# rockstaedt/DecentralOPF.jl

Measured on AMD Instinct MI355X. Metric: agent_subproblem_updates_per_sec, higher is better.
Workload: dtype f64

## Files before the change

decentralopf.jl_amd/csrc/dopf_api.hip:

```cpp
#include <algorithm>
#include <cmath>
#include <cstdarg>
#include <cstdio>
#include <cstdlib>
#include <cstring>
#include <numeric>
#include <string>
#include <vector>

#include "dopf_ctx.h"

using namespace dopf;

namespace {

#ifndef DOPF_UNROLL
#define DOPF_UNROLL 16
#endif
constexpr int kUnroll = DOPF_UNROLL, kMid = 4;
constexpr int kGraphIters[3] = {kUnroll, kMid, 1};
constexpr int kCheckEvery = 512;
thread_local char g_create_err[512];

}
// ... 318 lines not shown
};

Step make_step(const dopf_ctx *c, bool quiet, bool outside = false)
{
    const Plan &p = c->plan;
    const bool single = c->comm == nullptr && !outside;
    const XchgView *x = outside ? nullptr : comm_xchg(c);
    Step st{};
    st.xd = x && ((c->v.L == 0 && p.sliceDual) || c->tail_xchg) ? x : nullptr;
    st.like_single = single || st.xd != nullptr;
    st.comm_quiet = quiet && !st.like_single && x != nullptr && p.commQuiet;
    st.v = c->v;
    DevView &v = st.v;
    v.sliceDual = st.like_single && p.sliceDual;
    v.tail = st.like_single && c->v.tailDev && (c->comm == nullptr || c->tail_xchg) ? c->v.tailDev : nullptr;
    v.slackInDual = (st.like_single || st.comm_quiet) && p.slackDual;
    v.slackGlobal = st.comm_quiet ? 1 : 0;
    v.quiet = single && v.slackInDual && quiet;
    return st;
}

bool quiet_allowed(const dopf_ctx *c)
{
    return c->comm ? c->plan.commQuiet && comm_xchg(c) != nullptr && !c->tail_xchg : c->plan.quiet;
}

int settle_quiet(dopf_ctx *c, bool *parked)
{
    *parked = c->host_st.halt == 2;
    if (*parked) {
        HIPCHK(c, hipMemsetAsync(&c->v.st->halt, 0, sizeof(int), c->main));
        c->host_st.halt = 0;
        c->quiet = false;
        ++c->quiet_parked;
    } else if (!c->host_st.halt) {
        c->quiet = (c->comm ? c->plan.commQuiet : c->plan.quiet) && c->host_st.walk_last == 0;
    }
    return DOPF_OK;
}

enum { E_T0, E_T1, E_G0, E_G1, E_S0, E_S1, E_K0, E_K1, E_R1, E_D1, E_X0, E_X1, E_N };

void enqueue_local(dopf_ctx *c, const Step &st, const hipEvent_t *ev = nullptr)
{
    const DevView &v = st.v;
    const Plan &p = c->plan;
    auto mark = [&](int k, hipStream_t s) { if (ev) hipEventRecord(ev[k], s); };
    mark(E_T0, c->main);
    launch_tables(v, p, c->main);
    mark(E_T1, c->main);
    const bool fork = v.nGenItems > 0 && v.nStoItems > 0 && (c->q.flags & DOPF_F_OVERLAP_AGENTS);
    if (fork) {
        hipEventRecord(c->evFork, c->main);
        hipStreamWaitEvent(c->side, c->evFork, 0);
        mark(E_S0, c->side);
        launch_sto_update(v, p, c->side);
        mark(E_S1, c->side);
        hipEventRecord(c->evJoin, c->side);
    }
    mark(E_G0, c->main);
    if (p.fuseAgents) launch_agents_fused(v, p, c->main);
    else if (p.fuseNet) launch_net_agents(v, p, c->main);
    else launch_gen_update(v, p, c->main);
    mark(E_G1, c->main);
    if (fork) {
        hipStreamWaitEvent(c->main, c->evJoin, 0);
    } else {
        mark(E_S0, c->main);
        if (!p.fuseAgents && !p.fuseNet) launch_sto_update(v, p, c->main);
        mark(E_S1, c->main);
    }
    mark(E_K0, c->main);
    if (!v.tail && !v.quiet) launch_slack(v, c->main);
    mark(E_K1, c->main);
    if (!v.tail && !v.slackInDual) launch_reduce(v, p, c->main);
    mark(E_R1, c->main);
}

void enqueue_apply(dopf_ctx *c, const Step &st, const hipEvent_t *ev = nullptr)
{
    if (!st.v.tail) launch_dual(st.v, c->plan, c->main, st.xd);
    if (ev) for (int k : {E_D1, E_X0, E_X1}) hipEventRecord(ev[k], c->main);
}

int enqueue_iteration(dopf_ctx *c, bool quiet = false, const hipEvent_t *ev = nullptr)
{
    const Step st = make_step(c, quiet);
    enqueue_local(c, st, ev);
    if (st.comm_quiet) launch_xchg(c->v, *comm_xchg(c), c->main, true);
    else if (!st.like_single) { const int rc = comm_enqueue_allreduce(c); if (rc) return rc; }
    enqueue_apply(c, st, ev);
    return DOPF_OK;
}

int build_graph(dopf_ctx *c, int iters, hipGraphExec_t *out, bool quiet = false)
{
    hipGraph_t g = nullptr;
    HIPCHK(c, hipStreamBeginCapture(c->main, c->comm ? hipStreamCaptureModeThreadLocal : hipStreamCaptureModeRelaxed));
    int rc = DOPF_OK;
    for (int i = 0; i < iters && rc == DOPF_OK; ++i) rc = enqueue_iteration(c, quiet);
    const hipError_t ec = hipStreamEndCapture(c->main, &g);
    if (rc) { if (g) hipGraphDestroy(g); return rc; }
    if (ec != hipSuccess) return fail(c, DOPF_E_DEVICE, "hipStreamEndCapture: %s", hipGetErrorString(ec));
    hipError_t e = hipGraphInstantiate(out, g, nullptr, nullptr, 0);
    hipGraphDestroy(g);
    if (e != hipSuccess) return fail(c, DOPF_E_DEVICE, "hipGraphInstantiate: %s", hipGetErrorString(e));
    return DOPF_OK;
}

int build_graphs(dopf_ctx *c, bool quiet)
{
    dopf_ctx::Graphs &gs = c->graphs[quiet];
    for (int k = 0; k < 3; ++k)
        if (const int rc = build_graph(c, kGraphIters[k], &gs.g[k], quiet)) return rc;
    gs.valid = true;
// ... 292 lines not shown
        d.zeros(&v.part_U, NT * L); d.zeros(&v.part_K, NT * L); d.zeros(&v.node_dsum, NT);
        d.zeros(&v.walk_flag, LT); d.zeros(&v.walk_any, T); d.zeros(&v.tab_skip, T);
    }
    d.zeros(&v.part_ginj, (size_t)v.nGenItems * T); d.zeros(&v.part_gcost, v.nGenItems);
    d.zeros(&v.part_sinj, (size_t)v.nStoItems * T); d.zeros(&v.part_scost, v.nStoItems);
    d.zeros(&v.part_sinj_w, (size_t)v.nStoItems * T); d.zeros(&v.part_scost_w, v.nStoItems);
    if (L > 0) { d.upload(&v.row_of_pos, lo.row_of_pos); d.upload(&v.pos_of_row, lo.pos_of_row); }
    if (L > 0) d.zeros(&v.part_T, (size_t)v.rowsT * T);
    if (L > 0) d.zeros(&v.prev_node, NT);
    d.zeros(&v.nu_prev, (size_t)S * T); d.zeros(&v.nu_valid, S); d.zeros(&v.sto_fail, S);
    d.zeros(&v.item_fail, v.nStoItems);
    d.zeros(&v.part2, (size_t)N * v.reduceRB * T); d.zeros(&v.part2_cost, v.reduceRB);
    d.zeros(&v.reduce_ticket, (size_t)N * ((T + 31) / 32));
    d.zeros(&v.dual_ticket, 1);
    if (pl.tail) {
        d.zeros(&tvh.acc, (size_t)2 * kAccRep * tvh.accStride);
        tvh.expect = agent_blocks(v);
        TailView *tvd = nullptr;
        d.raw(&tvd, 1);
        if (d.rc) return d.rc;
        HIPCHK(c, hipMemcpy(tvd, &tvh, sizeof tvh, hipMemcpyHostToDevice));
        v.tailDev = tvd;
    }
    if (pl.wideNet) {
        std::vector<double> na(N);
        for (int n = 0; n < N; ++n)
            na[n] = (double)((lo.node_gen_beg[n + 1] - lo.node_gen_beg[n]) + (lo.node_sto_beg[n + 1] - lo.node_sto_beg[n]));
        d.upload(&v.node_na, na);
    }
    double *cons = nullptr;
    d.zeros(&cons, NT + 2 * LT + 1);
// ... 887 lines not shown
```

decentralopf.jl_amd/csrc/dopf_internal.h:

```cpp
#pragma once

#include <hip/hip_runtime.h>
#include <stddef.h>
#include <stdint.h>
#include <stdlib.h>

#include <type_traits>

#include "../../include/dopf.h"
#include "dopf_plan.h"
#include "ramp_dp.h"
#include "budget_root.h"
#include "central_rows.h"

namespace dopf {

struct Status {
    int iteration;
    int converged;
    int halt;
    int iters_total;
    unsigned long long solver_fail;
    unsigned long long dbg_scans, dbg_wave_loops, dbg_events;
    unsigned long long dbg_cyc[6];
    unsigned long long dbg_reason[4];
    unsigned long long resbits[3];
    unsigned long long resbits2[2][3];
    int walk_last;
    int res_set;
    double res[3];
    double total_cost;
    int xchg_timeout;
    int tail_timeout;
    int tail_par;
};

struct XchgView;
struct TailView {
    long long *acc;
    int accStride;
    int expect;
    double scaleInj, invInj, scaleCost, invCost;
    const XchgView *xchg;
};

struct DevView {
    const DevView *self;
    int N, L, T, G, S, M2;
    int maxNodeAgents;
    int nGenItems, nStoItems;
    int genTT, genR;
    int genRows;
// ... 197 lines not shown
void central_launch_iteration(const CentralView &c, const Plan &p, const DevView &vreduce, hipStream_t s);
void central_launch_metrics(const CentralView &c, const Plan &p, const DevView &vreduce, const double *XP, const double *XD, const double *XC,
                            const double *XE, const double *yb, const double *yf, const double *XR, const double *XQ, double scale, hipStream_t s);
void central_launch_scale_copy(double *dst, const double *src, double scale, size_t n, hipStream_t s);
constexpr int kCentralDiffBlocks = 256;
int central_diff_blocks(size_t n);
void central_launch_diff_sq(const double *a, const double *b, size_t n, double *part, hipStream_t s);
void central_launch_scale_copy_primal(const CentralView &c, const Plan &p, double scale, hipStream_t s);

inline int agent_blocks(const DevView &v) { return v.nStoItems + (v.genBlocks > 0 && !v.genSkip ? v.genBlocks : v.nGenItems); }

void launch_gen_update(const DevView &v, const Plan &p, hipStream_t s);
void launch_gen_ramp(const DevView &v, const Plan &p, hipStream_t s);
void launch_gen_ramp_net(const DevView &v, const Plan &p, hipStream_t s);
void launch_gen_budget(const DevView &v, const Plan &p, hipStream_t s);
void launch_sto_update(const DevView &v, const Plan &p, hipStream_t s);
void launch_net_agents(const DevView &v, const Plan &p, hipStream_t s);
void launch_agents_fused(const DevView &v, const Plan &p, hipStream_t s);
int debug_timeline(unsigned long long *out, int n);
hipError_t raise_lds_limits(const DevView &v, const Plan &p);
void launch_tables(const DevView &v, const Plan &p, hipStream_t s);
void launch_slack(const DevView &v, hipStream_t s);
void launch_reduce(const DevView &v, const Plan &p, hipStream_t s);
constexpr int kXchgMaxWorld = 16;
constexpr int kXchgChunk = 2048;
struct XchgView {
    int world, me, nchunks;
    int rs;
    unsigned long long n;
    unsigned long long timeout_ticks;
    double *data[kXchgMaxWorld];
    unsigned long long *flags[kXchgMaxWorld];
    double *sum[kXchgMaxWorld];
// ... 18 lines not shown
```

decentralopf.jl_amd/csrc/kernels_agents.hip:

```cpp
#include "dopf_internal.h"

namespace dopf {

#if defined(DOPF_STATS) || defined(DOPF_BLOCK_STAMPS)
__device__ unsigned long long g_timeline[8192 * 8 + 8192 * 8];
#endif
#if defined(DOPF_STATS) || defined(DOPF_BLOCK_STAMPS)
#define DOPF_BLOCK_ENTER() { if (threadIdx.x == 0 && blockIdx.x < 8192 * 4) g_timeline[32768 + 2 * blockIdx.x] = wall_clock64(); }
#define DOPF_BLOCK_EXIT() { __syncthreads(); if (threadIdx.x == 0 && blockIdx.x < 8192 * 4) g_timeline[32768 + 2 * blockIdx.x + 1] = wall_clock64(); }
#else
#define DOPF_BLOCK_ENTER()
#define DOPF_BLOCK_EXIT()
#endif
#ifdef DOPF_BLOCK_STAMPS
#define DOPF_TAIL_STAMP(i) { if (threadIdx.x == 0) g_timeline[(i)] = wall_clock64(); }
#else
#define DOPF_TAIL_STAMP(i)
#endif
#ifdef DOPF_STATS
#define DOPF_STAMP(i) { if (lane == 0 && rep == 0 && round == 0) { const int w_ = blk * 4 + (tid >> 6); if (w_ < 8192) g_timeline[w_ * 8 + (i)] = wall_clock64(); } }
#else
#define DOPF_STAMP(i)
#endif

// ... 141 lines not shown
            v.st->total_cost = ctot;
        }
    }
    for (int d = 32; d > 0; d >>= 1) rl = fmax(rl, __shfl_xor(rl, d));
    if ((tid & 63) == 0) wmaxT[tid >> 6] = rl;
    asm volatile("s_waitcnt lgkmcnt(0)\n\ts_barrier" ::: "memory");
    DOPF_TAIL_STAMP(3)
    if (tid == 0) {
        if (badT & 2) { v.st->xchg_timeout = 1; v.st->halt = 1; return; }
        if (badT) { v.st->tail_timeout = 1; v.st->halt = 1; return; }
        double r0 = 0.0;
        for (int q = 0; q < nth / 64; ++q) r0 = fmax(r0, wmaxT[q]);
        v.st->tail_par = par ^ 1;
        status_update(v, spre, r0, 0.0, 0.0);
    }
}

__device__ __forceinline__ void lin_coef(double w, double iw, double kap, double &ia, double &idet, double &s2)
{
    const double r2 = rcp64(w + 2.0 * kap);
    ia = rcp64(w + kap);
    idet = iw * r2;
    s2 = 2.0 * r2;
}

template <int BS, int FL = 4, bool AV = false, bool QC = false>
__device__ __forceinline__ void gen_lines_body(const DevView &v, const int item, const int TT, const int R)
{
    __shared__ double red[BS];
    const Item it = v.gen_items[item];
// ... 262 lines not shown
}

template <bool LINES, bool AV = false, bool QC = false>
__global__ __launch_bounds__(512) void k_gen_update(DevView v)
{
    gen_update_body<LINES, AV, QC>(v);
}

template <int BS, bool TAIL, bool LDS_ONLY = false>
__device__ __forceinline__ void gen_pair_sums(const DevView &v, const int blk, const int tid, const int r, const int tt,
                                              double acc0, double acc1, double cost, double (*red)[BS], double *wc)
{
    const int T = v.T, TT = v.genTT2, R = v.genR2;
    TailView tv{};
    int par = 0;
    if (TAIL) { tv = *v.tail; par = v.st->tail_par; }
    for (int d = 32; d > 0; d >>= 1) cost += __shfl_xor(cost, d);
    red[0][tid] = acc0; red[1][tid] = acc1;
    if ((tid & 63) == 0) wc[tid >> 6] = cost;
    if (LDS_ONLY) asm volatile("s_waitcnt lgkmcnt(0)\n\ts_barrier" ::: "memory");
    else __syncthreads();
    if (r == 0 && tt < TT) {
        double s0 = 0.0, s1 = 0.0;
        for (int q = 0; q < R; ++q) { s0 += red[0][q * TT + tt]; s1 += red[1][q * TT + tt]; }
        if (TAIL) {
            acc_add(tv, par, 2 * tt, s0, tv.scaleInj);
            acc_add(tv, par, 2 * tt + 1, s1, tv.scaleInj);
        } else {
            v.part_ginj[(size_t)blk * T + 2 * tt] = s0;
            v.part_ginj[(size_t)blk * T + 2 * tt + 1] = s1;
        }
// ... 14 lines not shown
    __shared__ double wc[BS / 64];
    Item it;
    if (v.genChunk > 0) { it.a0 = blk * v.genChunk; it.a1 = min(v.G, it.a0 + v.genChunk); it.node = 0; }
    else it = v.gen_items[blk];
    const int T = v.T, N = v.N, TT = v.genTT2, R = v.genR2;
    const int tid = threadIdx.x;
    const int r = tid / TT, tt = tid - r * TT;
    const double w = v.w_prox, gam = v.gamma;
    const double inv = 1.0 / (w + gam);
    double cost = 0.0, acc0 = 0.0, acc1 = 0.0;
    const double *ftab = nullptr;
    const int *prof = nullptr;
    if constexpr (AV) { ftab = *gen_avail_slot(v); prof = gen_prof(v); }
    if (r < R) {
        const int t = 2 * tt;
        const double sh0 = fma(gam, v.s[t], v.price[it.node + N * t]) * inv;
        const double sh1 = fma(gam, v.s[t + 1], v.price[it.node + N * (t + 1)]) * inv;
        double2 *P2 = reinterpret_cast<double2 *>(v.P);
        const size_t half = (size_t)(T >> 1);
        constexpr int GU = BS == 256 ? 6 : 4;
        for (int g0 = it.a0 + r; g0 < it.a1; g0 += GU * R) {
            double2 p0[GU], cp[GU];
            double mc[GU], pm[GU];
            int pr[GU];
#pragma unroll
            for (int u = 0; u < GU; ++u) {
                const int g = g0 + u * R < it.a1 ? g0 + u * R : g0;
                mc[u] = v.gen_mc[g]; pm[u] = v.gen_pmax[g];
                p0[u] = P2[(size_t)g * half + tt];
                if constexpr (AV) pr[u] = prof[g];
            }
            if constexpr (AV) {
// ... 19 lines not shown
}

template <int BS, bool TAIL, bool AV = false>
__device__ __forceinline__ bool gen_pair_stream(const DevView &v, const int first, const int stride)
{
    constexpr int GU = kGenStreamRows;
    __shared__ double red[2][BS];
    __shared__ double wc[BS / 64];
    const int halt = v.st->halt;
    const int T = v.T, N = v.N, TT = v.genTT2, R = v.genR2, nI = v.nGenItems, chunk = v.genChunk, G = v.G;
    const int tid = threadIdx.x;
    const int r = tid / TT, tt = tid - r * TT;
    const bool rowlane = r < R;
    const double gam = v.gamma, inv = 1.0 / (v.w_prox + gam);
    const int t2c = 2 * tt;
    const double sh0 = fma(gam, v.s[t2c], v.price[(size_t)N * t2c]) * inv;
    const double sh1 = fma(gam, v.s[t2c + 1], v.price[(size_t)N * (t2c + 1)]) * inv;
    if (first >= nI) return halt == 0;
    double2 *P2 = reinterpret_cast<double2 *>(v.P);
    const size_t half = (size_t)(T >> 1);
    double2 pa[GU], pb[GU];
    double mca[GU], pma[GU], mcb[GU], pmb[GU];
    int pra[GU], prb[GU];
    const double *ftab = nullptr;
    const int *prof = nullptr;
    if constexpr (AV) { ftab = *gen_avail_slot(v); prof = gen_prof(v); }
#define DOPF_GEN_LOAD(item, p, mc, pm, pr)                                                  \
    {                                                                                       \
        const int a0_ = (item) * chunk, a1_ = min(G, a0_ + chunk);                          \
        _Pragma("unroll") for (int u = 0; u < GU; ++u) {                                    \
            const int g_ = (rowlane && a0_ + r + u * R < a1_) ? a0_ + r + u * R : a0_;      \
            const double2 mp_ = v.gen_mp[g_];                                               \
// ... 56 lines not shown
__device__ __forceinline__ void gen_pair_skip_body(const DevView &v, const int blk)
{
    __shared__ double red[2][BS];
    __shared__ double wc[BS / 64], wlo[BS / 64], whi[BS / 64];
    __shared__ int flg[2][BS];
    const Item it = v.gen_items[blk];
    const int T = v.T, N = v.N, TT = v.genTT2, R = v.genR2;
    const int tid = threadIdx.x;
    const int r = tid / TT, tt = tid - r * TT;
    const double w = v.w_prox, gam = v.gamma;
    const double inv = 1.0 / (w + gam);
    double cost = 0.0, acc0 = 0.0, acc1 = 0.0;
    double sh0 = 0.0, sh1 = 0.0;
    if (r < R) {
        const int t = 2 * tt;
        sh0 = fma(gam, v.s[t], v.price[it.node + N * t]) * inv;
        sh1 = fma(gam, v.s[t + 1], v.price[it.node + N * (t + 1)]) * inv;
    }
    double lo = (r == 0 && tt < TT) ? fmin(sh0, sh1) : INFINITY, hi = (r == 0 && tt < TT) ? fmax(sh0, sh1) : -INFINITY;
    for (int d = 32; d > 0; d >>= 1) { lo = fmin(lo, __shfl_xor(lo, d)); hi = fmax(hi, __shfl_xor(hi, d)); }
    if ((tid & 63) == 0) { wlo[tid >> 6] = lo; whi[tid >> 6] = hi; }
    flg[0][tid] = 3; flg[1][tid] = 3;
    __syncthreads();
    double smin = wlo[0], smax = whi[0];
    for (int q = 1; q < BS / 64; ++q) { smin = fmin(smin, wlo[q]); smax = fmax(smax, whi[q]); }

    double2 *P2 = reinterpret_cast<double2 *>(v.P);
    const size_t half = (size_t)(T >> 1);
    const int nPass = (it.a1 - it.a0 + R - 1) / R;
    double mcN, pmN;
    int sttN, prN = -1;
    const double *ftab = nullptr;
// ... 377 lines not shown
        if (LINES) for (int t = tid; t < T; t += 256) v.part_T[(size_t)t * v.rowsT + it.row] = 0.0;
        else for (int t = tid; t < T; t += 256) v.part_sinj[(size_t)blk * T + t] = 0.0;
        if (tid == 0) v.part_scost[blk] = 0.0;
        return;
    }
    const double w = v.w_prox, gam = v.gamma;
    const double a0 = w + gam, ia0 = 1.0 / a0, idet0 = 1.0 / (a0 * a0 - gam * gam), s20 = 2.0 / (a0 + gam);
    const int tbase = li * NCH;

    double th0[NCH], accQ[NCH];
    double accCost = 0.0;
#pragma unroll
    for (int c = 0; c < NCH; ++c) {
        const int t = tbase + c;
        accQ[c] = 0.0;
        th0[c] = (!LINES && t < T) ? v.price[it.node + N * t] + gam * v.s[t] : 0.0;
    }
    double lp0[NCH], lkap[NCH];
    bool lin[NCH];
#pragma unroll
    for (int c = 0; c < NCH; ++c) {
        const int t = tbase + c;
        lin[c] = false; lp0[c] = 0.0; lkap[c] = 0.0;
        if (LINES && t < T) {
            const size_t at = (size_t)it.node + (size_t)N * t;
            const int m_ = v.tb_m[at];
            const double p0_ = v.tb_psi0[at], k_ = v.tb_slope[at * (v.M2 + 1)];
            if (m_ == 0) {
                lin[c] = true;
                lp0[c] = p0_;
                lkap[c] = k_;
// ... 243 lines not shown
            }
        }
    }

#pragma unroll
    for (int c = 0; c < NCH; ++c) red[(grp * LPS + li) * NCH + c] = accQ[c];
    redc[tid] = accCost;
    __syncthreads();
    if (grp == 0) {
#pragma unroll
        for (int c = 0; c < NCH; ++c) {
            const int t = tbase + c;
            if (t < T) {
                double sum = 0.0;
                for (int g2 = 0; g2 < NG; ++g2) sum += red[(g2 * LPS + li) * NCH + c];
                if (TAIL) { const TailView tv = *v.tail; acc_add(tv, v.st->tail_par, t, sum + v.part_sinj_w[(size_t)blk * T + t], tv.scaleInj); }
                else if (LINES) v.part_T[(size_t)t * v.rowsT + it.row] = sum;
                else v.part_sinj[(size_t)blk * T + t] = sum;
            }
        }
    }
    for (int sft = 128; sft > 0; sft >>= 1) {
        if (tid < sft) redc[tid] += redc[tid + sft];
        __syncthreads();
    }
    if (tid == 0) {
        if (TAIL) { const TailView tv = *v.tail; acc_add(tv, v.st->tail_par, T, redc[0] + v.part_scost_w[blk], tv.scaleCost); }
        else v.part_scost[blk] = redc[0];
    }
    if (fails) atomicAdd(&v.st->solver_fail, fails);
#ifdef DOPF_STATS
    if (st_scans) atomicAdd(&v.st->dbg_scans, st_scans);
    if (st_loops) atomicAdd(&v.st->dbg_wave_loops, st_loops);
    if (st_events) atomicAdd(&v.st->dbg_events, st_events);
#endif
}

template <int LPS, int NCH, bool LINES, int LV>
__global__ __launch_bounds__(256, 2) void k_sto_update(DevView v)
{
    if (v.st->halt) return;
    sto_cold_body<LPS, NCH, LINES, false, false, LV>(v, blockIdx.x, -1);
// ... 198 lines not shown
        const double iw = 1.0 / w;
        double run = li == 0 ? e0 : 0.0;
#pragma unroll
        for (int c = 0; c < NCH; ++c) {
            const int t = tbase + c;
            const bool ok = live && t < T;
            const size_t e = (size_t)s * T + (ok ? t : 0);
            const double d0 = ok ? v.D[e] : 0.0, c0 = ok ? v.C[e] : 0.0;
            const double nu_st = v.nu_prev[ok ? e : 0];
            nuv[c] = (ok && havenu) ? nu_st : 0.0;
            hint[c] = 0;
            dq[c] = EF ? be * c0 - al * d0 : c0 - d0;
            run += EF ? be * c0 - al * d0 : c0 - d0;
            if (LINES) { A0[c] = d0; B0[c] = c0; }
            else {
                const double th0 = t < T ? v.price[it.node + N * t] + gam * v.s[t] : 0.0;
                const double theta = th0 - gam * (d0 - c0);
                A0[c] = w * d0 - mc - theta; B0[c] = w * c0 - mc + theta;
                nuv[c] = (ok && havenu) ? nu_st - theta : 0.0;
            }
        }
        if (rep == 0 && halt) return -1;
        auto eval = [&](int c, double nu, double &dd, double &cc, double &s1) {
            const double nD = EF ? al * nu : nu, nC = EF ? be * nu : nu;
            if (!LINES) {
                box2(a0, gam, ia0, idet0, s20, A0[c] - nD, B0[c] + nC, pm, dd, cc, s1);
                if (EF) s1 = eff_slope(a0, gam, ia0, idet0, al, be, pm, dd, cc);
            } else if (lin[c]) {
                const double q0 = A0[c] - B0[c], theta = lp0[c] - lkap[c] * q0;
                double lia, lidet, ls2;
                lin_coef(w, iw, lkap[c], lia, lidet, ls2);
// ... 414 lines not shown
#undef DOPF_TIC
#undef DOPF_TOC

#pragma unroll
    for (int c = 0; c < NCH; ++c) red[(grp * LPS + li) * NCH + c] = accQ[c];
    __shared__ double wcostS[4];
    __shared__ int wfailS[4];
    {
        double cw = accCost;
        int fw = anyFail;
        for (int d = 32; d > 0; d >>= 1) { cw += __shfl_xor(cw, d); fw += __shfl_xor(fw, d); }
        if (lane == 0) { wcostS[tid >> 6] = cw; wfailS[tid >> 6] = fw; }
    }
    TailView tv{};
    int tpar = 0;
    if (TAIL) { tv = *v.tail; tpar = v.st->tail_par; }
    asm volatile("s_waitcnt lgkmcnt(0)\n\ts_barrier" ::: "memory");
    const int blockFail = wfailS[0] + wfailS[1] + wfailS[2] + wfailS[3];
    if (grp == 0) {
#pragma unroll
        for (int c = 0; c < NCH; ++c) {
            const int t = tbase + c;
            if (t < T) {
                double sum = 0.0;
                for (int g2 = 0; g2 < NG; ++g2) sum += red[(g2 * LPS + li) * NCH + c];
                if (TAIL && blockFail == 0) acc_add(tv, tpar, t, sum, tv.scaleInj);
                else if (LINES) v.part_T[(size_t)t * v.rowsT + it.row + 1] = sum;
                else v.part_sinj_w[(size_t)blk * T + t] = sum;
            }
        }
    }
// ... 90 lines not shown
        const int left = LEAN ? sto_lean_body<LPS, NCH, false, true, false>(v, si, v.st->halt)
                              : sto_warm_body<LPS, NCH, true, false, false, LV>(v, si, v.st->halt);
        if (left < 0) return;
        if (left == 0) {
            const int row = v.sto_items[si].row;
            for (int t = threadIdx.x; t < v.T; t += 256) v.part_T[(size_t)t * v.rowsT + row] = 0.0;
            if (threadIdx.x == 0) v.part_scost[si] = 0.0;
        } else {
            sto_cold_lines_call<LPS, NCH, LV>(v.self, si, left);
        }
    }
    DOPF_BLOCK_EXIT();
}

template <int LPS, int NCH, bool LINES, bool TAIL, bool FULLT, int LV = 0>
__global__ __launch_bounds__(256, 3) void k_sto(DevView v)
{
    if (TAIL && (int)blockIdx.x == v.nStoItems) { tail_block(v.self); return; }
    const int left = sto_warm_body<LPS, NCH, LINES, TAIL, FULLT, LV>(v, blockIdx.x, v.st->halt);
    if (left < 0) return;
    sto_cold_body<LPS, NCH, LINES, TAIL, FULLT, LV>(v, blockIdx.x, left);
}

template <int LPS, int NCH, bool SKIP, bool TAIL, bool FULLT, int LV = 0, bool AV = false>
__global__ __launch_bounds__(256, 3) void k_agents(DevView v)
{
    const int nS = v.nStoItems;
    DOPF_BLOCK_ENTER();
    if (TAIL && blockIdx.x == gridDim.x - 1) {
        tail_block(v.self);
    } else if (!SKIP && (int)blockIdx.x >= nS) {
        if (v.genBlocks > 0) gen_pair_stream<256, TAIL, AV>(v, blockIdx.x - nS, v.genBlocks);
        else gen_pair_body<256, TAIL, true, AV>(v, blockIdx.x - nS);
    } else {
        if ((int)blockIdx.x < nS) {
            const int left = sto_warm_body<LPS, NCH, false, TAIL, FULLT, LV>(v, blockIdx.x, v.st->halt);
            if (left >= 0) sto_cold_body<LPS, NCH, false, TAIL, FULLT, LV>(v, blockIdx.x, left);
        } else {
            if (v.st->halt) return;
            gen_pair_skip_body<256, TAIL, AV>(v, blockIdx.x - nS);
        }
    }
    DOPF_BLOCK_EXIT();
}

#ifndef DOPF_LEAN_STO_WAVES
#define DOPF_LEAN_STO_WAVES 3
#endif
template <int LPS, int NCH, bool TAIL, bool FULLT = true>
__global__ __launch_bounds__(256, DOPF_LEAN_STO_WAVES) void k_sto_l(DevView v)
{
    if (TAIL && (int)blockIdx.x == v.nStoItems) { tail_block(v.self); return; }
    const int left = sto_lean_body<LPS, NCH, TAIL, false, FULLT>(v, blockIdx.x, v.st->halt);
    if (left < 0) return;
    sto_cold_body<LPS, NCH, false, TAIL, FULLT>(v, blockIdx.x, left);
}

template <int LPS, int NCH, bool SKIP, bool TAIL, bool FULLT = true, bool AV = false>
__global__ __launch_bounds__(256, 3) void k_agents_l(DevView v)
{
    const int nS = v.nStoItems;
    DOPF_BLOCK_ENTER();
    if (TAIL && blockIdx.x == gridDim.x - 1) {
        tail_block(v.self);
    } else if (!SKIP && (int)blockIdx.x >= nS) {
        if (v.genBlocks > 0) gen_pair_stream<256, TAIL, AV>(v, blockIdx.x - nS, v.genBlocks);
        else gen_pair_body<256, TAIL, true, AV>(v, blockIdx.x - nS);
    } else {
        if ((int)blockIdx.x < nS) {
            const int left = sto_lean_body<LPS, NCH, TAIL, false, FULLT>(v, blockIdx.x, v.st->halt);
            if (left >= 0) sto_cold_body<LPS, NCH, false, TAIL, FULLT>(v, blockIdx.x, left);
        } else {
            if (v.st->halt) return;
            gen_pair_skip_body<256, TAIL, AV>(v, blockIdx.x - nS);
        }
    }
    DOPF_BLOCK_EXIT();
}

int debug_timeline(unsigned long long *out, int n)
{
#if defined(DOPF_STATS) || defined(DOPF_BLOCK_STAMPS)
    return hipMemcpyFromSymbol(out, HIP_SYMBOL(g_timeline), sizeof(unsigned long long) * (size_t)n) == hipSuccess ? 0 : -1;
#else
    (void)out; (void)n;
    return -1;
#endif
}

template <int LPS, int NCH>
static void launch_sto_t(const DevView &v, const Plan &p, hipStream_t s)
{
    constexpr int NC = NCH <= 3 ? NCH : 3;
    if (v.use_warm && v.L == 0) {
        const dim3 grid(v.nStoItems + (v.tail ? 1 : 0));
        with_bool(v.tail, [&](auto tail) { with_bool(v.T == LPS * NC, [&](auto full) {
            constexpr bool TL = decltype(tail)::value, FU = decltype(full)::value;
            if (p.stoLean) hipLaunchKernelGGL((k_sto_l<LPS, NC, TL, FU>), grid, dim3(256), 0, s, v);
            else with_lv(p.stoLV, [&](auto lv) { hipLaunchKernelGGL((k_sto<LPS, NC, false, TL, FU, decltype(lv)::value>), grid, dim3(256), 0, s, v); });
        }); });
        return;
    }
    if (v.use_warm) {
        if (p.stoLean) hipLaunchKernelGGL((k_sto_warm<LPS, NC, true, true>), dim3(v.nStoItems), dim3(256), 0, s, v);
        else with_lv(p.stoLV, [&](auto lv) { hipLaunchKernelGGL((k_sto_warm<LPS, NC, true, false, decltype(lv)::value>), dim3(v.nStoItems), dim3(256), 0, s, v); });
        return;
    }
    with_lv(p.stoLV, [&](auto lv) {
        constexpr int LV = decltype(lv)::value;
        if (v.L > 0) hipLaunchKernelGGL((k_sto_update<LPS, NCH, true, LV>), dim3(v.nStoItems), dim3(256), 0, s, v);
        else hipLaunchKernelGGL((k_sto_update<LPS, NCH, false, LV>), dim3(v.nStoItems), dim3(256), 0, s, v);
    });
}

template <int LPS, int NCH>
static void launch_agents_t(const DevView &v, const Plan &p, hipStream_t s)
{
    const dim3 grid(agent_blocks(v) + (v.tail ? 1 : 0));
    with_bool(v.genSkip, [&](auto skip) { with_bool(v.tail, [&](auto tail) { with_bool(v.T == LPS * NCH, [&](auto full) { with_bool(p.genAvail, [&](auto av) {
        constexpr bool SK = decltype(skip)::value, TL = decltype(tail)::value, FU = decltype(full)::value, AV = decltype(av)::value;
        if (p.stoLean) hipLaunchKernelGGL((k_agents_l<LPS, NCH, SK, TL, FU, AV>), grid, dim3(256), 0, s, v);
        else with_lv(p.stoLV, [&](auto lv) { hipLaunchKernelGGL((k_agents<LPS, NCH, SK, TL, FU, decltype(lv)::value, AV>), grid, dim3(256), 0, s, v); });
    }); }); }); });
}

void launch_agents_fused(const DevView &v, const Plan &p, hipStream_t s)
{
    with_sto_pair<kFusedPairs>(p, [&](auto lps, auto nch) { launch_agents_t<decltype(lps)::value, decltype(nch)::value>(v, p, s); });
}

void launch_net_agents(const DevView &v, const Plan &p, hipStream_t s)
{
    const dim3 grid(v.nStoItems + v.nGenItems);
    with_sto_pair<kFusedPairs>(p, [&](auto lps, auto nch) { with_bool(p.genAvail, [&](auto av) {
        constexpr int LPS = decltype(lps)::value, NCH = decltype(nch)::value;
        if constexpr (decltype(av)::value) {
            if (p.stoLean) hipLaunchKernelGGL((k_net_agents_av<LPS, NCH, true>), grid, dim3(256), 0, s, v);
            else with_lv(p.stoLV, [&](auto lv) { hipLaunchKernelGGL((k_net_agents_av<LPS, NCH, false, decltype(lv)::value>), grid, dim3(256), 0, s, v); });
        } else {
            if (p.stoLean) hipLaunchKernelGGL((k_net_agents<LPS, NCH, true>), grid, dim3(256), 0, s, v);
            else with_lv(p.stoLV, [&](auto lv) { hipLaunchKernelGGL((k_net_agents<LPS, NCH, false, decltype(lv)::value>), grid, dim3(256), 0, s, v); });
        }
    }); });
}

void launch_sto_update(const DevView &v, const Plan &p, hipStream_t s)
{
    if (v.nStoItems == 0) return;
    if (p.stoLong) {
        with_lv(p.stoLV, [&](auto lv) {
            constexpr int LV = decltype(lv)::value;
            if (v.L > 0) hipLaunchKernelGGL((k_sto_long<true, LV>), dim3(v.nStoItems), dim3(kLongBS), 0, s, v);
            else hipLaunchKernelGGL((k_sto_long<false, LV>), dim3(v.nStoItems), dim3(kLongBS), 0, s, v);
        });
        return;
    }
    with_sto_pair<kAllPairs>(p, [&](auto lps, auto nch) { launch_sto_t<decltype(lps)::value, decltype(nch)::value>(v, p, s); });
}

}
```

decentralopf.jl_amd/csrc/sto_lean.h:

```cpp
#pragma once
#include <type_traits>

namespace dopf {

template <class Tp>
__device__ __forceinline__ Tp *lz_at(Tp *base, unsigned byte_off)
{
    return reinterpret_cast<Tp *>(reinterpret_cast<char *>(const_cast<typename std::remove_const<Tp>::type *>(base)) + byte_off);
}

template <int CTRL>
__device__ __forceinline__ double lz_dpp(double x)
{
    const int lo = __builtin_amdgcn_update_dpp(0, __double2loint(x), CTRL, 0xF, 0xF, true);
    const int hi = __builtin_amdgcn_update_dpp(0, __double2hiint(x), CTRL, 0xF, 0xF, true);
    return __hiloint2double(hi, lo);
}
template <int CTRL>
__device__ __forceinline__ int lz_dppi(int x)
{
    return __builtin_amdgcn_update_dpp(0, x, CTRL, 0xF, 0xF, true);
}
template <int CTRL, bool ZERO_OK>
__device__ __forceinline__ double lz_dpp_id(double x, double idv)
// ... 166 lines not shown
                lin_coef(w, 1.0 / w, k_, iaL[c], idetL[c], s2L[c]);
            }
        }
        if (__syncthreads_or(nonlin)) return sto_warm_lines_call<LPS, NCH>(v.self, blk, halt);
    }

    double accQ[NCH];
    double accCost = 0.0;
    int anyFail = 0;
#pragma unroll
    for (int c = 0; c < NCH; ++c) accQ[c] = 0.0;
    __shared__ double th0L[TP];
    if (!LINES) {
        if (tid < LPS) {
#pragma unroll
            for (int c = 0; c < NCH; ++c) th0L[tbase + c] = LZ_IN(c) ? v.price[it.node + N * (tbase + c)] + gam * v.s[tbase + c] : 0.0;
        }
        __syncthreads();
    }
#ifdef DOPF_STATS
    unsigned long long st_rounds = 0, st_newton = 0, st_short = 0;
#endif
    const int nRep = (it.a1 - it.a0 + NG - 1) / NG;
    for (int rep = 0; rep < nRep; ++rep) {
        const int s = it.a0 + rep * NG + grp;
        const bool live = s < it.a1;
        const unsigned sl = live ? (unsigned)s : (unsigned)it.a0;
        const double mc = v.sto_mc[sl], pm = v.sto_pmax[sl], em = v.sto_emax[sl];
        const bool havenu = live && v.nu_valid[sl] != 0;
        double A0[NCH], B0[NCH], nuv[NCH], dq[NCH];
        double run = 0.0;
// ... 377 lines not shown
    __shared__ int wfailS[4];
    {
        double cw = accCost;
        int fw = anyFail;
        for (int d = 32; d > 0; d >>= 1) { cw += __shfl_xor(cw, d); fw += __shfl_xor(fw, d); }
        if (lane == 0) { wcostS[tid >> 6] = cw; wfailS[tid >> 6] = fw; }
        if (lane < LPS) {
#pragma unroll
            for (int c = 0; c < NCH; ++c) wsumS[tid >> 6][tbase + c] = accQ[c];
        }
    }
    const DevView *pf = v.self;
    asm volatile("" : "+s"(pf));
    TailView tv{};
    int tpar = 0;
    if (TAIL) { tv = *pf->tailDev; tpar = pf->st->tail_par; }
    asm volatile("s_waitcnt lgkmcnt(0)\n\ts_barrier" ::: "memory");
    const int blockFail = wfailS[0] + wfailS[1] + wfailS[2] + wfailS[3];
    if (tid < LPS) {
#pragma unroll
        for (int c = 0; c < NCH; ++c) {
            const int t = tbase + c;
            if (!LZ_IN(c)) continue;
            const double sum = ((wsumS[0][t] + wsumS[1][t]) + wsumS[2][t]) + wsumS[3][t];
            if (TAIL && blockFail == 0) acc_add(tv, tpar, t, sum, tv.scaleInj);
            else if (LINES) pf->part_T[(size_t)t * pf->rowsT + it.row + 1] = sum;
            else pf->part_sinj_w[(size_t)blk * T + t] = sum;
        }
    }
    if (tid == 0) {
        const double cw = ((wcostS[0] + wcostS[1]) + wcostS[2]) + wcostS[3];
// ... 17 lines not shown
```

Measured before the change: 2.160 billion.

## Defer tail dual update into next iteration's agent kernel prologue within graphs

Within a captured single-device graph with fused agents, the tail block no longer performs the dual/price update at the end of each iteration. Instead every agent block recomputes the price and slack from the triple-buffered fixed-point accumulators in its own prologue and caches them in LDS. A single finish kernel at the end of the graph writes the final duals and status. This removes a serialized grid-wide tail step per iteration, at the cost of redundant per-block reduction work, a third accumulator set, and the tail path being disabled for storage problems with T above 192.

```diff
diff --git a/decentralopf.jl_amd/csrc/dopf_api.hip b/decentralopf.jl_amd/csrc/dopf_api.hip
--- a/decentralopf.jl_amd/csrc/dopf_api.hip
+++ b/decentralopf.jl_amd/csrc/dopf_api.hip
@@ -356,6 +356,7 @@
     DevView &v = st.v;
     v.sliceDual = st.like_single && p.sliceDual;
     v.tail = st.like_single && c->v.tailDev && (c->comm == nullptr || c->tail_xchg) ? c->v.tailDev : nullptr;
+    if (v.tail && v.nStoItems > 0 && v.T > kTailStoT) v.tail = nullptr;
     v.slackInDual = (st.like_single || st.comm_quiet) && p.slackDual;
     v.slackGlobal = st.comm_quiet ? 1 : 0;
     v.quiet = single && v.slackInDual && quiet;
@@ -383,7 +384,7 @@
 
 enum { E_T0, E_T1, E_G0, E_G1, E_S0, E_S1, E_K0, E_K1, E_R1, E_D1, E_X0, E_X1, E_N };
 
-void enqueue_local(dopf_ctx *c, const Step &st, const hipEvent_t *ev = nullptr)
+void enqueue_local(dopf_ctx *c, const Step &st, const hipEvent_t *ev = nullptr, int step = -1)
 {
     const DevView &v = st.v;
     const Plan &p = c->plan;
@@ -396,12 +397,12 @@
         hipEventRecord(c->evFork, c->main);
         hipStreamWaitEvent(c->side, c->evFork, 0);
         mark(E_S0, c->side);
-        launch_sto_update(v, p, c->side);
+        launch_sto_update(v, p, c->side, step);
         mark(E_S1, c->side);
         hipEventRecord(c->evJoin, c->side);
     }
     mark(E_G0, c->main);
-    if (p.fuseAgents) launch_agents_fused(v, p, c->main);
+    if (p.fuseAgents) launch_agents_fused(v, p, c->main, step);
     else if (p.fuseNet) launch_net_agents(v, p, c->main);
     else launch_gen_update(v, p, c->main);
     mark(E_G1, c->main);
@@ -409,7 +410,7 @@
         hipStreamWaitEvent(c->main, c->evJoin, 0);
     } else {
         mark(E_S0, c->main);
-        if (!p.fuseAgents && !p.fuseNet) launch_sto_update(v, p, c->main);
+        if (!p.fuseAgents && !p.fuseNet) launch_sto_update(v, p, c->main, step);
         mark(E_S1, c->main);
     }
     mark(E_K0, c->main);
@@ -425,22 +426,30 @@
     if (ev) for (int k : {E_D1, E_X0, E_X1}) hipEventRecord(ev[k], c->main);
 }
 
-int enqueue_iteration(dopf_ctx *c, bool quiet = false, const hipEvent_t *ev = nullptr)
+int enqueue_iteration(dopf_ctx *c, bool quiet = false, const hipEvent_t *ev = nullptr, int step = -1)
 {
     const Step st = make_step(c, quiet);
-    enqueue_local(c, st, ev);
+    enqueue_local(c, st, ev, step);
     if (st.comm_quiet) launch_xchg(c->v, *comm_xchg(c), c->main, true);
     else if (!st.like_single) { const int rc = comm_enqueue_allreduce(c); if (rc) return rc; }
     enqueue_apply(c, st, ev);
     return DOPF_OK;
 }
 
+bool tail_deferred(const dopf_ctx *c, const Step &st)
+{
+    return st.v.tail != nullptr && c->comm == nullptr && !c->tail_xchg && c->plan.fuseAgents;
+}
+
 int build_graph(dopf_ctx *c, int iters, hipGraphExec_t *out, bool quiet = false)
 {
     hipGraph_t g = nullptr;
+    const Step st0 = make_step(c, quiet);
+    const bool deferred = tail_deferred(c, st0);
     HIPCHK(c, hipStreamBeginCapture(c->main, c->comm ? hipStreamCaptureModeThreadLocal : hipStreamCaptureModeRelaxed));
     int rc = DOPF_OK;
-    for (int i = 0; i < iters && rc == DOPF_OK; ++i) rc = enqueue_iteration(c, quiet);
+    for (int i = 0; i < iters && rc == DOPF_OK; ++i) rc = enqueue_iteration(c, quiet, nullptr, deferred ? i : -1);
+    if (deferred && rc == DOPF_OK) launch_tail_finish(st0.v, iters, c->main);
     const hipError_t ec = hipStreamEndCapture(c->main, &g);
     if (rc) { if (g) hipGraphDestroy(g); return rc; }
     if (ec != hipSuccess) return fail(c, DOPF_E_DEVICE, "hipStreamEndCapture: %s", hipGetErrorString(ec));
@@ -763,7 +772,7 @@
     d.zeros(&v.reduce_ticket, (size_t)N * ((T + 31) / 32));
     d.zeros(&v.dual_ticket, 1);
     if (pl.tail) {
-        d.zeros(&tvh.acc, (size_t)2 * kAccRep * tvh.accStride);
+        d.zeros(&tvh.acc, (size_t)3 * kAccRep * tvh.accStride + 2 * (size_t)T);
         tvh.expect = agent_blocks(v);
         TailView *tvd = nullptr;
         d.raw(&tvd, 1);
diff --git a/decentralopf.jl_amd/csrc/dopf_internal.h b/decentralopf.jl_amd/csrc/dopf_internal.h
--- a/decentralopf.jl_amd/csrc/dopf_internal.h
+++ b/decentralopf.jl_amd/csrc/dopf_internal.h
@@ -33,9 +33,11 @@
     int xchg_timeout;
     int tail_timeout;
     int tail_par;
+    int tail_stop;
 };
 
 struct XchgView;
+constexpr int kTailStoT = 192;
 struct TailView {
     long long *acc;
     int accStride;
@@ -263,9 +265,10 @@
 void launch_gen_ramp(const DevView &v, const Plan &p, hipStream_t s);
 void launch_gen_ramp_net(const DevView &v, const Plan &p, hipStream_t s);
 void launch_gen_budget(const DevView &v, const Plan &p, hipStream_t s);
-void launch_sto_update(const DevView &v, const Plan &p, hipStream_t s);
+void launch_sto_update(const DevView &v, const Plan &p, hipStream_t s, int step = -1);
 void launch_net_agents(const DevView &v, const Plan &p, hipStream_t s);
-void launch_agents_fused(const DevView &v, const Plan &p, hipStream_t s);
+void launch_agents_fused(const DevView &v, const Plan &p, hipStream_t s, int step = -1);
+void launch_tail_finish(const DevView &v, int J, hipStream_t s);
 int debug_timeline(unsigned long long *out, int n);
 hipError_t raise_lds_limits(const DevView &v, const Plan &p);
 void launch_tables(const DevView &v, const Plan &p, hipStream_t s);
diff --git a/decentralopf.jl_amd/csrc/kernels_agents.hip b/decentralopf.jl_amd/csrc/kernels_agents.hip
--- a/decentralopf.jl_amd/csrc/kernels_agents.hip
+++ b/decentralopf.jl_amd/csrc/kernels_agents.hip
@@ -179,6 +179,171 @@
         v.st->tail_par = par ^ 1;
         status_update(v, spre, r0, 0.0, 0.0);
     }
+}
+
+template <int BS>
+struct TailLds {
+    static_assert(BS == 256, "the launches with storage blocks");
+    static constexpr int kT = kTailStoT;
+    double price[kT], s[kT];
+    double wmax[BS / 64];
+    int set;
+};
+template <int BS>
+__device__ __forceinline__ TailLds<BS> &tail_lds()
+{
+    __shared__ TailLds<BS> l;
+    return l;
+}
+
+__device__ __forceinline__ double *tail_spare(const TailView &tv, int T, int which)
+{
+    return reinterpret_cast<double *>(tv.acc + (size_t)3 * kAccRep * tv.accStride) + (size_t)which * T;
+}
+
+template <int BS>
+__device__ __forceinline__ int tail_prologue(const DevView &v, const int step)
+{
+    TailLds<BS> &l = tail_lds<BS>();
+    const int tid = threadIdx.x, T = v.T;
+    const int halt = v.st->halt, par = v.st->tail_par;
+    if (step <= 0) {
+        for (int t = tid; t < T; t += BS) { l.price[t] = v.price[t]; l.s[t] = v.s[t]; }
+        if (tid == 0) l.set = par;
+        __syncthreads();
+        return halt ? 1 : 0;
+    }
+    const TailView tv = *v.tail;
+    const int it = v.st->iteration + step - 1, conv0 = v.st->converged;
+    const int rset = (par + step + 2) % 3;
+    const double *lamOld = ((step - 1) & 1) ? tail_spare(tv, T, 0) : v.lam;
+    constexpr int HR = kAccRep / 2;
+    const int half = tid & 1;
+    double rl = 0.0;
+    for (int t0 = 0; t0 < T; t0 += BS / 2) {
+        const int t = t0 + (tid >> 1);
+        const bool act = t < T;
+        const int tc = act ? t : 0;
+        const double dem = v.demand[tc], lam_old = lamOld[tc];
+        const unsigned long long *base = reinterpret_cast<const unsigned long long *>(tv.acc) +
+                                         ((size_t)rset * kAccRep + (size_t)half * HR) * tv.accStride + tc;
+        unsigned long long x[HR];
+#pragma unroll
+        for (int r = 0; r < HR; ++r) x[r] = base[(size_t)r * tv.accStride];
+        long long sum = 0;
+#pragma unroll
+        for (int r = 0; r < HR; ++r) sum += (long long)(x[r] & ~kAccCntMask) >> kAccCntBits;
+        sum += __shfl_xor(sum, 1);
+        if (act && !half) {
+            const double xsum = (double)sum * tv.invInj;
+            const double tot = xsum;
+            const double xi = tot - dem;
+            const double ln = lam_old + v.gamma * xi;
+            l.price[t] = ln;
+            l.s[t] = xi;
+            rl = fmax(rl, fabs(ln - lam_old));
+        }
+    }
+    for (int d = 32; d > 0; d >>= 1) rl = fmax(rl, __shfl_xor(rl, d));
+    if ((tid & 63) == 0) l.wmax[tid >> 6] = rl;
+    if (tid == 0) l.set = (par + step) % 3;
+    __syncthreads();
+    double r0 = 0.0;
+    for (int q = 0; q < BS / 64; ++q) r0 = fmax(r0, l.wmax[q]);
+    int conv = conv0;
+    if (it != 1) conv = (r0 < v.eps) && (0.0 < v.eps) && (0.0 < v.eps);
+    const bool stop = conv || (v.max_iters > 0 && it + 1 > v.max_iters);
+    return halt ? 1 : (stop ? 2 : 0);
+}
+
+template <int BS>
+__device__ __forceinline__ void tail_writer(const DevView &v, const int step)
+{
+    const int verdict = tail_prologue<BS>(v, step);
+    if (verdict == 1) return;
+    const int tid = threadIdx.x, T = v.T;
+    if (verdict == 2) {
+        if (tid == 0) { v.st->tail_stop = step; v.st->halt = 1; }
+        return;
+    }
+    const TailView tv = *v.tail;
+    if (step > 0) {
+        const TailLds<BS> &l = tail_lds<BS>();
+        double *lamN = (step & 1) ? tail_spare(tv, T, 0) : v.lam, *sN = (step & 1) ? tail_spare(tv, T, 1) : v.s;
+        for (int t = tid; t < T; t += BS) { lamN[t] = l.price[t]; sN[t] = l.s[t]; }
+    }
+    unsigned long long *z = reinterpret_cast<unsigned long long *>(tv.acc) + (size_t)((v.st->tail_par + step + 1) % 3) * kAccRep * tv.accStride;
+    for (int i = tid; i < kAccRep * tv.accStride; i += BS) __hip_atomic_store(z + i, 0ull, __ATOMIC_RELAXED, __HIP_MEMORY_SCOPE_AGENT);
+}
+
+__global__ __launch_bounds__(256) void k_tail_finish(DevView v, int J)
+{
+    __shared__ double wmaxT[4];
+    Status *st = v.st;
+    const int stopAt = st->tail_stop, halt = st->halt;
+    if (stopAt == 0 && halt) return;
+    const int jj = stopAt ? stopAt : J;
+    const TailView tv = *v.tail;
+    const int tid = threadIdx.x, T = v.T, par = st->tail_par;
+    StatusPre spre;
+    spre.iteration = st->iteration + jj - 1; spre.converged = st->converged; spre.iters_total = st->iters_total + jj - 1;
+    const int rset = (par + jj + 2) % 3;
+    const bool spare = ((jj - 1) & 1) != 0;
+    const double *lamOld = spare ? tail_spare(tv, T, 0) : v.lam, *sOld = spare ? tail_spare(tv, T, 1) : v.s;
+    constexpr int HR = kAccRep / 2;
+    const int half = tid & 1;
+    double rl = 0.0;
+    for (int t0 = 0; t0 <= T; t0 += 128) {
+        const int t = t0 + (tid >> 1);
+        const bool act = t <= T;
+        const int tc = t < T ? t : 0;
+        const double dem = v.demand[tc], lam_old = lamOld[tc], s_old = sOld[tc];
+        const unsigned long long *base = reinterpret_cast<const unsigned long long *>(tv.acc) +
+                                         ((size_t)rset * kAccRep + (size_t)half * HR) * tv.accStride + (act ? t : 0);
+        unsigned long long x[HR];
+#pragma unroll
+        for (int r = 0; r < HR; ++r)
+            x[r] = __hip_atomic_load(base + (size_t)r * tv.accStride, __ATOMIC_RELAXED, __HIP_MEMORY_SCOPE_AGENT);
+        long long isum = 0;
+#pragma unroll
+        for (int r = 0; r < HR; ++r) isum += (long long)(x[r] & ~kAccCntMask) >> kAccCntBits;
+        isum += __shfl_xor(isum, 1);
+        if (!act || half) continue;
+        const double xsum = t < T ? (double)isum * tv.invInj : (double)isum * tv.invCost;
+        if (t < T) {
+            const double tot = xsum;
+            const double xi = tot - dem;
+            v.cons[t] = tot;
+            v.inj[t] = xi;
+            v.s_used[t] = s_old;
+            v.s[t] = xi;
+            const double ln = lam_old + v.gamma * xi;
+            v.lam_used[t] = lam_old;
+            v.lam[t] = ln;
+            v.price[t] = ln;
+            rl = fmax(rl, fabs(ln - lam_old));
+        } else {
+            const double ctot = xsum;
+            v.cons[T] = ctot;
+            st->total_cost = ctot;
+        }
+    }
+    for (int d = 32; d > 0; d >>= 1) rl = fmax(rl, __shfl_xor(rl, d));
+    if ((tid & 63) == 0) wmaxT[tid >> 6] = rl;
+    __syncthreads();
+    unsigned long long *z = reinterpret_cast<unsigned long long *>(tv.acc);
+    for (int i = tid; i < 3 * kAccRep * tv.accStride; i += 256) __hip_atomic_store(z + i, 0ull, __ATOMIC_RELAXED, __HIP_MEMORY_SCOPE_AGENT);
+    if (tid == 0) {
+        double r0 = 0.0;
+        for (int q = 0; q < 4; ++q) r0 = fmax(r0, wmaxT[q]);
+        st->tail_stop = 0;
+        status_update(v, spre, r0, 0.0, 0.0);
+    }
+}
+
+void launch_tail_finish(const DevView &v, int J, hipStream_t s)
+{
+    hipLaunchKernelGGL(k_tail_finish, dim3(1), dim3(256), 0, s, v, J);
 }
 
 __device__ __forceinline__ void lin_coef(double w, double iw, double kap, double &ia, double &idet, double &s2)
@@ -471,7 +636,7 @@
     const int T = v.T, TT = v.genTT2, R = v.genR2;
     TailView tv{};
     int par = 0;
-    if (TAIL) { tv = *v.tail; par = v.st->tail_par; }
+    if (TAIL) { tv = *v.tail; par = BS == 256 ? tail_lds<256>().set : v.st->tail_par; }
     for (int d = 32; d > 0; d >>= 1) cost += __shfl_xor(cost, d);
     red[0][tid] = acc0; red[1][tid] = acc1;
     if ((tid & 63) == 0) wc[tid >> 6] = cost;
@@ -516,8 +681,8 @@
     if constexpr (AV) { ftab = *gen_avail_slot(v); prof = gen_prof(v); }
     if (r < R) {
         const int t = 2 * tt;
-        const double sh0 = fma(gam, v.s[t], v.price[it.node + N * t]) * inv;
-        const double sh1 = fma(gam, v.s[t + 1], v.price[it.node + N * (t + 1)]) * inv;
+        const double sh0 = (TAIL && BS == 256) ? fma(gam, tail_lds<256>().s[t], tail_lds<256>().price[t]) * inv : fma(gam, v.s[t], v.price[it.node + N * t]) * inv;
+        const double sh1 = (TAIL && BS == 256) ? fma(gam, tail_lds<256>().s[t + 1], tail_lds<256>().price[t + 1]) * inv : fma(gam, v.s[t + 1], v.price[it.node + N * (t + 1)]) * inv;
         double2 *P2 = reinterpret_cast<double2 *>(v.P);
         const size_t half = (size_t)(T >> 1);
         constexpr int GU = BS == 256 ? 6 : 4;
@@ -567,8 +732,9 @@
     const bool rowlane = r < R;
     const double gam = v.gamma, inv = 1.0 / (v.w_prox + gam);
     const int t2c = 2 * tt;
-    const double sh0 = fma(gam, v.s[t2c], v.price[(size_t)N * t2c]) * inv;
-    const double sh1 = fma(gam, v.s[t2c + 1], v.price[(size_t)N * (t2c + 1)]) * inv;
+    const double sh0 = (TAIL && BS == 256) ? fma(gam, tail_lds<256>().s[t2c], tail_lds<256>().price[t2c]) * inv : fma(gam, v.s[t2c], v.price[(size_t)N * t2c]) * inv;
+    const double sh1 = (TAIL && BS == 256) ? fma(gam, tail_lds<256>().s[t2c + 1], tail_lds<256>().price[t2c + 1]) * inv
+                            : fma(gam, v.s[t2c + 1], v.price[(size_t)N * (t2c + 1)]) * inv;
     if (first >= nI) return halt == 0;
     double2 *P2 = reinterpret_cast<double2 *>(v.P);
     const size_t half = (size_t)(T >> 1);
@@ -655,8 +821,8 @@
     double sh0 = 0.0, sh1 = 0.0;
     if (r < R) {
         const int t = 2 * tt;
-        sh0 = fma(gam, v.s[t], v.price[it.node + N * t]) * inv;
-        sh1 = fma(gam, v.s[t + 1], v.price[it.node + N * (t + 1)]) * inv;
+        sh0 = (TAIL && BS == 256) ? fma(gam, tail_lds<256>().s[t], tail_lds<256>().price[t]) * inv : fma(gam, v.s[t], v.price[it.node + N * t]) * inv;
+        sh1 = (TAIL && BS == 256) ? fma(gam, tail_lds<256>().s[t + 1], tail_lds<256>().price[t + 1]) * inv : fma(gam, v.s[t + 1], v.price[it.node + N * (t + 1)]) * inv;
     }
     double lo = (r == 0 && tt < TT) ? fmin(sh0, sh1) : INFINITY, hi = (r == 0 && tt < TT) ? fmax(sh0, sh1) : -INFINITY;
     for (int d = 32; d > 0; d >>= 1) { lo = fmin(lo, __shfl_xor(lo, d)); hi = fmax(hi, __shfl_xor(hi, d)); }
@@ -1064,7 +1230,8 @@
     for (int c = 0; c < NCH; ++c) {
         const int t = tbase + c;
         accQ[c] = 0.0;
-        th0[c] = (!LINES && t < T) ? v.price[it.node + N * t] + gam * v.s[t] : 0.0;
+        if (TAIL) th0[c] = t < T ? tail_lds<256>().price[t] + gam * tail_lds<256>().s[t] : 0.0;
+        else th0[c] = (!LINES && t < T) ? v.price[it.node + N * t] + gam * v.s[t] : 0.0;
     }
     double lp0[NCH], lkap[NCH];
     bool lin[NCH];
@@ -1338,7 +1505,7 @@
             if (t < T) {
                 double sum = 0.0;
                 for (int g2 = 0; g2 < NG; ++g2) sum += red[(g2 * LPS + li) * NCH + c];
-                if (TAIL) { const TailView tv = *v.tail; acc_add(tv, v.st->tail_par, t, sum + v.part_sinj_w[(size_t)blk * T + t], tv.scaleInj); }
+                if (TAIL) { const TailView tv = *v.tail; acc_add(tv, tail_lds<256>().set, t, sum + v.part_sinj_w[(size_t)blk * T + t], tv.scaleInj); }
                 else if (LINES) v.part_T[(size_t)t * v.rowsT + it.row] = sum;
                 else v.part_sinj[(size_t)blk * T + t] = sum;
             }
@@ -1349,7 +1516,7 @@
         __syncthreads();
     }
     if (tid == 0) {
-        if (TAIL) { const TailView tv = *v.tail; acc_add(tv, v.st->tail_par, T, redc[0] + v.part_scost_w[blk], tv.scaleCost); }
+        if (TAIL) { const TailView tv = *v.tail; acc_add(tv, tail_lds<256>().set, T, redc[0] + v.part_scost_w[blk], tv.scaleCost); }
         else v.part_scost[blk] = redc[0];
     }
     if (fails) atomicAdd(&v.st->solver_fail, fails);
@@ -1578,7 +1745,7 @@
             run += EF ? be * c0 - al * d0 : c0 - d0;
             if (LINES) { A0[c] = d0; B0[c] = c0; }
             else {
-                const double th0 = t < T ? v.price[it.node + N * t] + gam * v.s[t] : 0.0;
+                const double th0 = t < T ? (TAIL ? tail_lds<256>().price[t] + gam * tail_lds<256>().s[t] : v.price[it.node + N * t] + gam * v.s[t]) : 0.0;
                 const double theta = th0 - gam * (d0 - c0);
                 A0[c] = w * d0 - mc - theta; B0[c] = w * c0 - mc + theta;
                 nuv[c] = (ok && havenu) ? nu_st - theta : 0.0;
@@ -2023,7 +2190,7 @@
     }
     TailView tv{};
     int tpar = 0;
-    if (TAIL) { tv = *v.tail; tpar = v.st->tail_par; }
+    if (TAIL) { tv = *v.tail; tpar = tail_lds<256>().set; }
     asm volatile("s_waitcnt lgkmcnt(0)\n\ts_barrier" ::: "memory");
     const int blockFail = wfailS[0] + wfailS[1] + wfailS[2] + wfailS[3];
     if (grp == 0) {
@@ -2144,21 +2311,24 @@
 }
 
 template <int LPS, int NCH, bool LINES, bool TAIL, bool FULLT, int LV = 0>
-__global__ __launch_bounds__(256, 3) void k_sto(DevView v)
-{
-    if (TAIL && (int)blockIdx.x == v.nStoItems) { tail_block(v.self); return; }
+__global__ __launch_bounds__(256, 3) void k_sto(DevView v, int step)
+{
+    if (TAIL && (int)blockIdx.x == v.nStoItems) { if (step < 0) tail_block(v.self); else tail_writer<256>(v, step); return; }
+    if (TAIL && tail_prologue<256>(v, step)) return;
     const int left = sto_warm_body<LPS, NCH, LINES, TAIL, FULLT, LV>(v, blockIdx.x, v.st->halt);
     if (left < 0) return;
     sto_cold_body<LPS, NCH, LINES, TAIL, FULLT, LV>(v, blockIdx.x, left);
 }
 
 template <int LPS, int NCH, bool SKIP, bool TAIL, bool FULLT, int LV = 0, bool AV = false>
-__global__ __launch_bounds__(256, 3) void k_agents(DevView v)
+__global__ __launch_bounds__(256, 3) void k_agents(DevView v, int step)
 {
     const int nS = v.nStoItems;
     DOPF_BLOCK_ENTER();
     if (TAIL && blockIdx.x == gridDim.x - 1) {
-        tail_block(v.self);
+        if (step < 0) tail_block(v.self);
+        else tail_writer<256>(v, step);
+    } else if (TAIL && tail_prologue<256>(v, step)) {
     } else if (!SKIP && (int)blockIdx.x >= nS) {
         if (v.genBlocks > 0) gen_pair_stream<256, TAIL, AV>(v, blockIdx.x - nS, v.genBlocks);
         else gen_pair_body<256, TAIL, true, AV>(v, blockIdx.x - nS);
@@ -2178,21 +2348,24 @@
 #define DOPF_LEAN_STO_WAVES 3
 #endif
 template <int LPS, int NCH, bool TAIL, bool FULLT = true>
-__global__ __launch_bounds__(256, DOPF_LEAN_STO_WAVES) void k_sto_l(DevView v)
-{
-    if (TAIL && (int)blockIdx.x == v.nStoItems) { tail_block(v.self); return; }
+__global__ __launch_bounds__(256, DOPF_LEAN_STO_WAVES) void k_sto_l(DevView v, int step)
+{
+    if (TAIL && (int)blockIdx.x == v.nStoItems) { if (step < 0) tail_block(v.self); else tail_writer<256>(v, step); return; }
+    if (TAIL && tail_prologue<256>(v, step)) return;
     const int left = sto_lean_body<LPS, NCH, TAIL, false, FULLT>(v, blockIdx.x, v.st->halt);
     if (left < 0) return;
     sto_cold_body<LPS, NCH, false, TAIL, FULLT>(v, blockIdx.x, left);
 }
 
 template <int LPS, int NCH, bool SKIP, bool TAIL, bool FULLT = true, bool AV = false>
-__global__ __launch_bounds__(256, 3) void k_agents_l(DevView v)
+__global__ __launch_bounds__(256, 3) void k_agents_l(DevView v, int step)
 {
     const int nS = v.nStoItems;
     DOPF_BLOCK_ENTER();
     if (TAIL && blockIdx.x == gridDim.x - 1) {
-        tail_block(v.self);
+        if (step < 0) tail_block(v.self);
+        else tail_writer<256>(v, step);
+    } else if (TAIL && tail_prologue<256>(v, step)) {
     } else if (!SKIP && (int)blockIdx.x >= nS) {
         if (v.genBlocks > 0) gen_pair_stream<256, TAIL, AV>(v, blockIdx.x - nS, v.genBlocks);
         else gen_pair_body<256, TAIL, true, AV>(v, blockIdx.x - nS);
@@ -2219,15 +2392,15 @@
 }
 
 template <int LPS, int NCH>
-static void launch_sto_t(const DevView &v, const Plan &p, hipStream_t s)
+static void launch_sto_t(const DevView &v, const Plan &p, hipStream_t s, int step)
 {
     constexpr int NC = NCH <= 3 ? NCH : 3;
     if (v.use_warm && v.L == 0) {
         const dim3 grid(v.nStoItems + (v.tail ? 1 : 0));
         with_bool(v.tail, [&](auto tail) { with_bool(v.T == LPS * NC, [&](auto full) {
             constexpr bool TL = decltype(tail)::value, FU = decltype(full)::value;
-            if (p.stoLean) hipLaunchKernelGGL((k_sto_l<LPS, NC, TL, FU>), grid, dim3(256), 0, s, v);
-            else with_lv(p.stoLV, [&](auto lv) { hipLaunchKernelGGL((k_sto<LPS, NC, false, TL, FU, decltype(lv)::value>), grid, dim3(256), 0, s, v); });
+            if (p.stoLean) hipLaunchKernelGGL((k_sto_l<LPS, NC, TL, FU>), grid, dim3(256), 0, s, v, step);
+            else with_lv(p.stoLV, [&](auto lv) { hipLaunchKernelGGL((k_sto<LPS, NC, false, TL, FU, decltype(lv)::value>), grid, dim3(256), 0, s, v, step); });
         }); });
         return;
     }
@@ -2244,19 +2417,19 @@
 }
 
 template <int LPS, int NCH>
-static void launch_agents_t(const DevView &v, const Plan &p, hipStream_t s)
+static void launch_agents_t(const DevView &v, const Plan &p, hipStream_t s, int step)
 {
     const dim3 grid(agent_blocks(v) + (v.tail ? 1 : 0));
     with_bool(v.genSkip, [&](auto skip) { with_bool(v.tail, [&](auto tail) { with_bool(v.T == LPS * NCH, [&](auto full) { with_bool(p.genAvail, [&](auto av) {
         constexpr bool SK = decltype(skip)::value, TL = decltype(tail)::value, FU = decltype(full)::value, AV = decltype(av)::value;
-        if (p.stoLean) hipLaunchKernelGGL((k_agents_l<LPS, NCH, SK, TL, FU, AV>), grid, dim3(256), 0, s, v);
-        else with_lv(p.stoLV, [&](auto lv) { hipLaunchKernelGGL((k_agents<LPS, NCH, SK, TL, FU, decltype(lv)::value, AV>), grid, dim3(256), 0, s, v); });
+        if (p.stoLean) hipLaunchKernelGGL((k_agents_l<LPS, NCH, SK, TL, FU, AV>), grid, dim3(256), 0, s, v, step);
+        else with_lv(p.stoLV, [&](auto lv) { hipLaunchKernelGGL((k_agents<LPS, NCH, SK, TL, FU, decltype(lv)::value, AV>), grid, dim3(256), 0, s, v, step); });
     }); }); }); });
 }
 
-void launch_agents_fused(const DevView &v, const Plan &p, hipStream_t s)
-{
-    with_sto_pair<kFusedPairs>(p, [&](auto lps, auto nch) { launch_agents_t<decltype(lps)::value, decltype(nch)::value>(v, p, s); });
+void launch_agents_fused(const DevView &v, const Plan &p, hipStream_t s, int step)
+{
+    with_sto_pair<kFusedPairs>(p, [&](auto lps, auto nch) { launch_agents_t<decltype(lps)::value, decltype(nch)::value>(v, p, s, step); });
 }
 
 void launch_net_agents(const DevView &v, const Plan &p, hipStream_t s)
@@ -2274,7 +2447,7 @@
     }); });
 }
 
-void launch_sto_update(const DevView &v, const Plan &p, hipStream_t s)
+void launch_sto_update(const DevView &v, const Plan &p, hipStream_t s, int step)
 {
     if (v.nStoItems == 0) return;
     if (p.stoLong) {
@@ -2285,7 +2458,7 @@
         });
         return;
     }
-    with_sto_pair<kAllPairs>(p, [&](auto lps, auto nch) { launch_sto_t<decltype(lps)::value, decltype(nch)::value>(v, p, s); });
-}
-
-}
+    with_sto_pair<kAllPairs>(p, [&](auto lps, auto nch) { launch_sto_t<decltype(lps)::value, decltype(nch)::value>(v, p, s, step); });
+}
+
+}
diff --git a/decentralopf.jl_amd/csrc/sto_lean.h b/decentralopf.jl_amd/csrc/sto_lean.h
--- a/decentralopf.jl_amd/csrc/sto_lean.h
+++ b/decentralopf.jl_amd/csrc/sto_lean.h
@@ -204,7 +204,10 @@
     if (!LINES) {
         if (tid < LPS) {
 #pragma unroll
-            for (int c = 0; c < NCH; ++c) th0L[tbase + c] = LZ_IN(c) ? v.price[it.node + N * (tbase + c)] + gam * v.s[tbase + c] : 0.0;
+            for (int c = 0; c < NCH; ++c) {
+                if (TAIL) th0L[tbase + c] = LZ_IN(c) ? tail_lds<256>().price[tbase + c] + gam * tail_lds<256>().s[tbase + c] : 0.0;
+                else th0L[tbase + c] = LZ_IN(c) ? v.price[it.node + N * (tbase + c)] + gam * v.s[tbase + c] : 0.0;
+            }
         }
         __syncthreads();
     }
@@ -612,7 +615,7 @@
     asm volatile("" : "+s"(pf));
     TailView tv{};
     int tpar = 0;
-    if (TAIL) { tv = *pf->tailDev; tpar = pf->st->tail_par; }
+    if (TAIL) { tv = *pf->tailDev; tpar = tail_lds<256>().set; }
     asm volatile("s_waitcnt lgkmcnt(0)\n\ts_barrier" ::: "memory");
     const int blockFail = wfailS[0] + wfailS[1] + wfailS[2] + wfailS[3];
     if (tid < LPS) {
```

After: 2.065 billion. 4.4% lower.
